# tbennun/capital

Hardware: NVIDIA H100
Metric: cholesky_tflops_fp64 (higher is better)
Workload: dtype f64

## Files before the change

capital_b200/csrc/common.cuh:

```cuda
#pragma once
#include <cuda.h>
#include <cuda_runtime.h>
#include <stdint.h>
#include <stdio.h>
#include <string.h>
#include <string>
#include <vector>
#include <map>
#include "../../include/capital_b200.h"

#define CAP_CUDA(call)                                                                                    \
  do {                                                                                                     \
    cudaError_t e__ = (call);                                                                              \
    if (e__ != cudaSuccess) {                                                                              \
      ctx->set_error(std::string(#call) + ": " + cudaGetErrorString(e__) + " (" + __FILE__ + ":" +         \
                     std::to_string(__LINE__) + ")");                                                      \
      return CAPITAL_ERR_CUDA;                                                                             \
    }                                                                                                      \
  } while (0)

#define CAP_TRY(call)                                  \
  do {                                                 \
    capital_status_t s__ = (call);                     \
    if (s__ != CAPITAL_OK) return s__;                 \
// ... 47 lines not shown
  int64_t tf32_min_k = 256;
  int64_t tf32_launches = 0;
  double tf32_flops = 0.0;
  std::vector<cudaEvent_t> prof_pool;
  size_t prof_used = 0;
  std::vector<ProfRec> prof_recs;
  capital_status_t prof_event(cudaEvent_t* out) {
    if (prof_used == prof_pool.size()) {
      cudaEvent_t e;
      if (cudaEventCreate(&e) != cudaSuccess) { err = "cudaEventCreate failed"; return CAPITAL_ERR_CUDA; }
      prof_pool.push_back(e);
    }
    *out = prof_pool[prof_used++];
    return CAPITAL_OK;
  }

  struct TlRec { cudaEvent_t e0, e1; int sid, kind; double a, b, c; };
  bool timeline = false;
  std::vector<TlRec> tl;
  std::vector<cudaEvent_t> tl_pool;
  size_t tl_used = 0;
  int stream_id(cudaStream_t st) const;
  int tl_begin(cudaStream_t st, int kind, double a = 0, double b = 0, double c = 0);
  void tl_end(cudaStream_t st, int idx);

  void set_error(const std::string& s) { err = s; }
  capital_status_t workspace(const std::string& name, size_t bytes, void** out);
};

capital_status_t gemm_tn_init(capital_ctx* ctx);
capital_status_t leaf_init(capital_ctx* ctx);
capital_status_t gemm_probe_dmma(capital_ctx* ctx, double* tflops, double* ms);

constexpr int GEMM_NCLS_MAX = 2;
constexpr int GEMM_XPEERS_MAX = 3;
struct GemmXDev {
  int mode, c, z;
  double* Cpeer[GEMM_XPEERS_MAX];
};
struct GemmOperands {
  int ncls = 1;
  const double* A[GEMM_NCLS_MAX] = {nullptr, nullptr};
  const double* B[GEMM_NCLS_MAX] = {nullptr, nullptr};
  int64_t lda = 0, ldb = 0;
};
capital_status_t gemm_tn_x(capital_ctx* ctx, cudaStream_t st, int64_t m, int64_t n, int64_t k, double alpha, const GemmOperands& ops,
                           double beta, double* C, int64_t ldc, int flags, int noff, const GemmXDev* x);
capital_status_t gemm_tn(capital_ctx* ctx, cudaStream_t st, int64_t m, int64_t n, int64_t k, double alpha, const double* A,
                         int64_t lda, const double* B, int64_t ldb, double beta, double* C, int64_t ldc, int flags);

capital_status_t gemm_tn_off(capital_ctx* ctx, cudaStream_t st, int64_t m, int64_t n, int64_t k, double alpha, const double* A,
                             int64_t lda, const double* B, int64_t ldb, double beta, double* C, int64_t ldc, int flags, int noff);
capital_status_t gemm_tn_splitk(capital_ctx* ctx, cudaStream_t st, int64_t m, int64_t n, int64_t k, double alpha, const double* A,
                                int64_t lda, const double* B, int64_t ldb, double* C, int64_t ldc, int flags);
capital_status_t gemm_tn_t(capital_ctx* ctx, cudaStream_t st, int64_t m, int64_t n, int64_t k, double alpha, const double* A, int64_t lda,
                           const double* B, int64_t ldb, double* C, int64_t ldc, double* Ct, int64_t ldct, int flags);

capital_status_t gemm_tf32_init(capital_ctx* ctx);
capital_status_t gemm_tn_tf32(capital_ctx* ctx, cudaStream_t st, int64_t m, int64_t n, int64_t k, double alpha, const double* A, int64_t lda,
                              const double* B, int64_t ldb, double beta, double* C, int64_t ldc, int flags, int passes);
capital_status_t gemm_tn_tf32_x(capital_ctx* ctx, cudaStream_t st, int64_t m, int64_t n, int64_t k, double alpha, const GemmOperands& ops,
                                double beta, double* C, int64_t ldc, int flags, int noff, int passes);
static inline bool trailing_uses_tf32(const capital_ctx* ctx, int64_t k) { return ctx->trailing_mode != 0 && k >= ctx->tf32_min_k; }

capital_status_t transpose_block(capital_ctx* ctx, cudaStream_t st, int64_t rows, int64_t cols, const double* src,
                                 int64_t lds, double* dst, int64_t ldd, double scale);
capital_status_t copy_block(capital_ctx* ctx, cudaStream_t st, int64_t rows, int64_t cols, const double* src, int64_t lds,
                            double* dst, int64_t ldd);
capital_status_t zero_block(capital_ctx* ctx, cudaStream_t st, int64_t rows, int64_t cols, double* dst, int64_t ldd);
capital_status_t zero_band(capital_ctx* ctx, cudaStream_t st, int64_t n, double* a, int64_t ld);
capital_status_t pack_upper(capital_ctx* ctx, cudaStream_t st, int64_t n, const double* src, int64_t lds, double* packed,
                            int zero_diag, int64_t col_begin = 0, int64_t col_end = -1);
capital_status_t unpack_upper(capital_ctx* ctx, cudaStream_t st, int64_t n, const double* packed, double* dst, int64_t ldd);
capital_status_t triu_copy(capital_ctx* ctx, cudaStream_t st, int64_t n, const double* src, int64_t lds, double* dst,
                           int64_t ldd, int zero_diag);
capital_status_t gen_symmetric(capital_ctx* ctx, cudaStream_t st, double* A, int64_t ld, int64_t lrows, int64_t lcols,
                               int64_t n_global, int x, int y, int d, int diag_dom);
capital_status_t gen_random(capital_ctx* ctx, cudaStream_t st, double* A, int64_t ld, int64_t lrows, int64_t lcols,
                            int64_t pad_rows, int64_t pad_cols, int64_t key);
capital_status_t sumsq_block(capital_ctx* ctx, cudaStream_t st, int64_t rows, int64_t cols, const double* a, int64_t ld,
                             int upper_mode, int x, int y, int d, double* out);
capital_status_t sub_identity_local(capital_ctx* ctx, cudaStream_t st, int64_t n, double* a, int64_t ld);

constexpr int LEAF_MAX = 64;
constexpr int BASECASE_MAX = 512;
capital_status_t basecase_cholinv(capital_ctx* ctx, cudaStream_t st, int nb, double* W, int64_t ldw, double* R, int64_t ldr,
                                  double* Ri, int64_t ldri, double* RiT, int64_t ldrit);
capital_status_t leaf_cholinv(capital_ctx* ctx, cudaStream_t st, int nb, const double* W, int64_t ldw, double* R, int64_t ldr,
                              double* Ri, int64_t ldri, double* RiT, int64_t ldrit);

struct CholinvHooks {
  void* user;
  capital_status_t (*need_cols)(void* user, cudaStream_t st, int64_t col_end);
  capital_status_t (*left_done)(void* user, cudaStream_t st, int64_t col_end, int depth);
  int64_t (*cols_waited)(void* user);
  capital_status_t (*right_done)(void* user, cudaStream_t st);
  capital_status_t (*inv_cols)(void* user, cudaStream_t st, int64_t col_end);
};
capital_status_t cholinv_local(capital_ctx* ctx, cudaStream_t st, int64_t n, double* W, int64_t ldw, double* R, int64_t ldr,
                               double* Ri, int64_t ldri, double* RiT, int64_t ldrit, bool complete_top, int64_t bc, int split,
                               const CholinvHooks* hooks = nullptr, bool allow_side = true);

static inline int64_t round_up(int64_t a, int64_t b) { return (a + b - 1) / b * b; }
static inline bool cholinv_node_splits(int64_t n, int64_t bc, int split) { return n > bc && (n >> split) >= split && (n >> split) > 0; }
static inline int64_t ceil_div(int64_t a, int64_t b) { return (a + b - 1) / b; }
```

capital_b200/csrc/gemm_tn.cu:

```cuda
#include "common.cuh"
#include <algorithm>

namespace {

struct GemmParams {
  int M, N, K;
  int rowoffA, rowoffB;
  int flags;
  int noff;
  int ksplit;
  int ncls;
  int gm, gn;
  double alpha, beta;
  double* C;
  long long ldc;
  double* Ct;
  long long ldct;
  double* kpart;
  long long kstride, ldk;
  int no_c;
  GemmXDev x;
};

struct GemmMaps {
  CUtensorMap a[GEMM_NCLS_MAX];
  CUtensorMap b[GEMM_NCLS_MAX];
};

__device__ __forceinline__ uint32_t smem_u32(const void* p) { return (uint32_t)__cvta_generic_to_shared(p); }

__device__ __forceinline__ void mbar_init(uint32_t bar, uint32_t count) {
  asm volatile("mbarrier.init.shared::cta.b64 [%0], %1;" ::"r"(bar), "r"(count) : "memory");
}
__device__ __forceinline__ void mbar_wait(uint32_t bar, uint32_t parity) {
  uint32_t ok;
  do {
    asm volatile(
        "{\n\t.reg .pred p;\n\t"
        "mbarrier.try_wait.parity.shared::cta.b64 p, [%1], %2;\n\t"
        "selp.u32 %0, 1, 0, p;\n\t}"
        : "=r"(ok)
        : "r"(bar), "r"(parity)
        : "memory");
  } while (!ok);
}
__device__ __forceinline__ void mbar_arrive(uint32_t bar) {
  asm volatile("mbarrier.arrive.shared::cta.b64 _, [%0];" ::"r"(bar) : "memory");
}
__device__ __forceinline__ void mbar_expect_tx(uint32_t bar, uint32_t bytes) {
  asm volatile("mbarrier.arrive.expect_tx.shared::cta.b64 _, [%0], %1;" ::"r"(bar), "r"(bytes) : "memory");
}
__device__ __forceinline__ void tma_load_2d(uint32_t dst, const CUtensorMap* map, uint32_t bar, int c0, int c1) {
  asm volatile(
      "cp.async.bulk.tensor.2d.shared::cluster.global.mbarrier::complete_tx::bytes [%0], [%1, {%3, %4}], [%2];" ::"r"(dst),
      "l"(map), "r"(bar), "r"(c0), "r"(c1)
      : "memory");
}
__device__ __forceinline__ void dmma16816(double& c0, double& c1, double& c2, double& c3, const double2 (&a0)[2], const double2 (&a1)[2],
                                          const double2 (&b)[2]) {
  asm("mma.sync.aligned.m16n8k16.row.col.f64.f64.f64.f64 {%0,%1,%2,%3}, {%4,%5,%6,%7,%8,%9,%10,%11}, {%12,%13,%14,%15}, {%0,%1,%2,%3};"
      : "+d"(c0), "+d"(c1), "+d"(c2), "+d"(c3)
      : "d"(a0[0].x), "d"(a1[0].x), "d"(a0[0].y), "d"(a1[0].y), "d"(a0[1].x), "d"(a1[1].x), "d"(a0[1].y), "d"(a1[1].y),
        "d"(b[0].x), "d"(b[0].y), "d"(b[1].x), "d"(b[1].y));
}

constexpr int BK = 16;

template <int BM, int BN, int WM, int WN, int STAGES, int MINB, int RC, int RP, int XMODE>
__global__ void __launch_bounds__(((BM / WM) * (BN / WN) + 4) * 32, MINB)
    gemm_tn_kernel(const __grid_constant__ GemmMaps maps, const GemmParams p) {
  constexpr int NWM = BM / WM, NWN = BN / WN, NCW = NWM * NWN;
  constexpr int FM = WM / 8, FN = WN / 8;
  static_assert(FM % 2 == 0, "DMMA.16x8x16 fragments pair the 8-row blocks of a warp tile");
  constexpr int A_BYTES = BM * 128, B_BYTES = BN * 128, STAGE_BYTES = A_BYTES + B_BYTES;

  extern __shared__ uint8_t smem_raw[];
  const int flags = p.flags;
  const int gm = p.gm, gn = p.gn;
  const int lin = (int)(blockIdx.x + gridDim.x * blockIdx.y);
  int tm, tn;
  if (flags & CAPITAL_GEMM_A_UPPER) { tm = gm - 1 - lin / gn; tn = lin % gn; }
  else if (flags & CAPITAL_GEMM_B_UPPER) { tn = gn - 1 - lin / gm; tm = lin % gm; }
  else if (flags & CAPITAL_GEMM_A_LOWER) { tm = lin / gn; tn = lin % gn; }
  else if (flags & CAPITAL_GEMM_B_LOWER) { tn = lin / gm; tm = lin % gm; }
  else { tm = lin % gm; tn = lin / gm; }
  if (XMODE == 2 && (tn % p.x.c) != p.x.z) return;
  const int m0 = tm * BM, n0 = tn * BN;
  const int n0g = n0 + p.noff;
  if ((flags & CAPITAL_GEMM_C_UPPER) && m0 > n0g + BN - 1) return;

  int kb = 0, ke = p.K;
  if (flags & CAPITAL_GEMM_A_UPPER) ke = min(ke, m0 + BM);
  if (flags & CAPITAL_GEMM_A_LOWER) kb = max(kb, m0);
  if (flags & CAPITAL_GEMM_B_UPPER) ke = min(ke, n0g + BN);
  if (flags & CAPITAL_GEMM_B_LOWER) kb = max(kb, n0g);
  kb &= ~(BK - 1);
  int nk = ke > kb ? (ke - kb + BK - 1) / BK : 0;
  if (nk == 0 && p.beta == 1.0 && p.ksplit <= 1) return;
  if (p.ksplit > 1) {
    const int per = (nk + p.ksplit - 1) / p.ksplit;
    const int t0 = min(nk, (int)blockIdx.z * per), t1 = min(nk, t0 + per);
    kb += t0 * BK;
    nk = t1 - t0;
    if (nk == 0) return;
  }
  const int niter = nk * p.ncls;

  const uint32_t raw_u32 = smem_u32(smem_raw);
  uint8_t* smem = smem_raw + (((raw_u32 + 1023u) & ~1023u) - raw_u32);
  const uint32_t smem_base = smem_u32(smem);
  const uint32_t full0 = smem_base + STAGES * STAGE_BYTES;
  const uint32_t empty0 = full0 + STAGES * 8;

  const int warp = threadIdx.x >> 5, lane = threadIdx.x & 31;
  if (threadIdx.x == 0) {
    for (int s = 0; s < STAGES; s++) {
      mbar_init(full0 + s * 8, 1);
      mbar_init(empty0 + s * 8, NCW);
    }
    asm volatile("fence.mbarrier_init.release.cluster;" ::: "memory");
    asm volatile("fence.proxy.async.shared::cta;" ::: "memory");
  }
  __syncthreads();

  if (warp >= NCW) {
    if (RC > 0) asm volatile("setmaxnreg.dec.sync.aligned.u32 %0;" ::"n"(RP));
    if (warp == NCW && lane == 0) {
      int it = 0;
      for (int cls = 0; cls < p.ncls; cls++) {
        const CUtensorMap* ma = cls ? &maps.a[1] : &maps.a[0];
        const CUtensorMap* mb = cls ? &maps.b[1] : &maps.b[0];
        for (int j = 0; j < nk; j++, it++) {
          const int s = it % STAGES;
          const uint32_t ph = (it / STAGES) & 1;
          mbar_wait(empty0 + s * 8, ph ^ 1);
          mbar_expect_tx(full0 + s * 8, STAGE_BYTES);
          const int kk = kb + j * BK;
          tma_load_2d(smem_base + s * STAGE_BYTES, ma, full0 + s * 8, p.rowoffA + kk, m0);
          tma_load_2d(smem_base + s * STAGE_BYTES + A_BYTES, mb, full0 + s * 8, p.rowoffB + kk, n0);
        }
      }
    }
    return;
  }

  if (RC > 0) asm volatile("setmaxnreg.inc.sync.aligned.u32 %0;" ::"n"(RC));
  const int wm = warp % NWM, wn = warp / NWM;
  const int g = lane >> 2, q = lane & 3;
// ... 336 lines not shown
```

capital_b200/csrc/leaf.cu:

```cuda
#include "common.cuh"
#include <cooperative_groups.h>
#include <stdlib.h>
#include <type_traits>
namespace cg = cooperative_groups;

namespace {
constexpr int LD = LEAF_MAX + 1;
constexpr int TLD = 68;
constexpr int TILE_DOUBLES = 64 * TLD;
constexpr int BC_CLUSTER = 8;

__device__ __forceinline__ double fast_rsqrt(double d) {
  if (!(d > 1e-30 && d < 1e30)) return rsqrt(d);
  double y = (double)rsqrtf((float)d);
  const double h = 0.5 * d;
  y = y * fma(-h, y * y, 1.5);
  y = y * fma(-h, y * y, 1.5);
  return y;
}

__device__ void leaf_factor_invert(int nb, double* __restrict__ a, double* __restrict__ r, double* __restrict__ t, int* info,
                                   int pivot_base) {
  const int tid = threadIdx.x, tx = tid & 15, ty = tid >> 4;
  for (int k = 0; k < nb; k++) {
    if (tid < 64 && tid >= k && tid < nb) {
      double d = a[k + k * LD];
      if (!(d > 0.0)) {
        if (tid == k) atomicCAS(info, 0, pivot_base + k + 1);
        d = 1.0;
      }
      const double rs = rsqrt(d);
      r[k + tid * LD] = (tid == k) ? d * rs : a[k + tid * LD] * rs;
    }
    __syncthreads();
#pragma unroll
    for (int ia = 0; ia < 4; ia++) {
      const int i = ty + 16 * ia;
      if (i > k && i < nb) {
        const double ri = r[k + i * LD];
#pragma unroll
        for (int jb = 0; jb < 4; jb++) {
          const int j = tx + 16 * jb;
          if (j >= i && j < nb) a[i + j * LD] -= ri * r[k + j * LD];
        }
      }
    }
    __syncthreads();
  }
#pragma unroll
  for (int ia = 0; ia < 4; ia++) {
    const int i = ty + 16 * ia;
#pragma unroll
    for (int jb = 0; jb < 4; jb++) {
      const int j = tx + 16 * jb;
      if (i < nb && j < nb) {
        if (i > j) r[i + j * LD] = 0.0;
        a[i + j * LD] = (i == j) ? 1.0 / r[i + i * LD] : 0.0;
      }
    }
  }
  __syncthreads();
  int lg = 0;
  for (int bs = 1; bs < nb; bs <<= 1, lg++) {
    const int span = 2 * bs;
    const int npairs = (nb + span - 1) / span;
    const int per = bs * bs, total = npairs * per;
    for (int idx = tid; idx < total; idx += 256) {
      const int p = idx >> (2 * lg), e = idx & (per - 1);
      const int li = e & (bs - 1), lj = e >> lg;
      const int o = p * span, i = o + li, j = o + bs + lj;
      if (j < nb) {
        double s = 0.0;
        const int kend = o + bs;
        for (int k = i; k < kend; k++) s += a[i + k * LD] * r[k + j * LD];
        t[i + j * LD] = s;
      }
    }
    __syncthreads();
    for (int idx = tid; idx < total; idx += 256) {
      const int p = idx >> (2 * lg), e = idx & (per - 1);
      const int li = e & (bs - 1), lj = e >> lg;
      const int o = p * span, i = o + li, j = o + bs + lj;
      if (j < nb) {
        double s = 0.0;
        for (int k = o + bs; k <= j; k++) s += t[i + k * LD] * a[k + j * LD];
        a[i + j * LD] = -s;
      }
    }
    __syncthreads();
  }
}

__device__ __forceinline__ void leaf_load(int nb, const double* W, long long ldw, double* __restrict__ a) {
  for (int idx = threadIdx.x; idx < nb * nb; idx += 256) {
    const int i = idx % nb, j = idx / nb;
    a[i + j * LD] = (i <= j) ? __ldcg(W + i + (long long)j * ldw) : 0.0;
  }
}
__device__ __forceinline__ void leaf_store(int nb, const double* a, const double* r, double* __restrict__ R,
                                           long long ldr, double* __restrict__ Ri, long long ldri, double* __restrict__ RiT,
                                           long long ldrit) {
  for (int idx = threadIdx.x; idx < nb * nb; idx += 256) {
    const int i = idx % nb, j = idx / nb;
    R[i + (long long)j * ldr] = r[i + j * LD];
    Ri[i + (long long)j * ldri] = a[i + j * LD];
  }
  if (RiT != nullptr) {
    for (int idx = threadIdx.x; idx < nb * nb; idx += 256) {
      const int j = idx % nb, i = idx / nb;
      RiT[j + (long long)i * ldrit] = a[i + j * LD];
    }
  }
}

__global__ void __launch_bounds__(256, 1)
    leaf_kernel(int nb, const double* W, long long ldw, double* __restrict__ R, long long ldr, double* __restrict__ Ri,
                long long ldri, double* __restrict__ RiT, long long ldrit, int* __restrict__ info) {
  extern __shared__ double sm[];
  double* a = sm;
  double* r = sm + LEAF_MAX * LD;
  double* t = sm + 2 * LEAF_MAX * LD;
  leaf_load(nb, W, ldw, a);
  __syncthreads();
  leaf_factor_invert(nb, a, r, t, info, 0);
  leaf_store(nb, a, r, R, ldr, Ri, ldri, RiT, ldrit);
}

__device__ __forceinline__ void dmma884(double& c0, double& c1, double a, double b) {
  asm("mma.sync.aligned.m8n8k4.row.col.f64.f64.f64.f64 {%0,%1}, {%2}, {%3}, {%0,%1};" : "+d"(c0), "+d"(c1) : "d"(a), "d"(b));
}
__device__ __forceinline__ void tile_load(double* __restrict__ dst, const double* src, long long ld) {
  const int k2 = (threadIdx.x & 31) * 2, c0 = threadIdx.x >> 5;
  double2 v[8];
#pragma unroll
  for (int r = 0; r < 8; r++) v[r] = __ldcg(reinterpret_cast<const double2*>(src + k2 + (long long)(c0 + 8 * r) * ld));
#pragma unroll
  for (int r = 0; r < 8; r++) *reinterpret_cast<double2*>(dst + (c0 + 8 * r) * TLD + k2) = v[r];
}
__device__ __forceinline__ void tile_mma(double (&acc)[4][2][2], const double* As, const double* Bs) {
  const int lane = threadIdx.x & 31, w = threadIdx.x >> 5, g = lane >> 2, q = lane & 3;
  const double* ap = As + ((w & 1) * 32 + g) * TLD + q;
  const double* bp = Bs + ((w >> 1) * 16 + g) * TLD + q;
#pragma unroll 4
  for (int k0 = 0; k0 < 64; k0 += 4) {
    double af[4], bf[2];
#pragma unroll
    for (int i = 0; i < 4; i++) af[i] = ap[i * 8 * TLD + k0];
#pragma unroll
    for (int j = 0; j < 2; j++) bf[j] = bp[j * 8 * TLD + k0];
#pragma unroll
    for (int i = 0; i < 4; i++)
#pragma unroll
      for (int j = 0; j < 2; j++) dmma884(acc[i][j][0], acc[i][j][1], af[i], bf[j]);
  }
}
__device__ __forceinline__ void acc_zero(double (&acc)[4][2][2]) {
#pragma unroll
  for (int i = 0; i < 4; i++)
#pragma unroll
    for (int j = 0; j < 2; j++) acc[i][j][0] = acc[i][j][1] = 0.0;
}
#define TILE_ROW(i) ((w & 1) * 32 + (i) * 8 + g)
#define TILE_COL(j, e) ((w >> 1) * 16 + (j) * 8 + 2 * q + (e))
__device__ __forceinline__ void acc_to_smem_colmajor(const double (&acc)[4][2][2], double* __restrict__ sC, double scale) {
  const int lane = threadIdx.x & 31, w = threadIdx.x >> 5, g = lane >> 2, q = lane & 3;
#pragma unroll
  for (int i = 0; i < 4; i++)
#pragma unroll
    for (int j = 0; j < 2; j++)
#pragma unroll
      for (int e = 0; e < 2; e++) sC[TILE_COL(j, e) * TLD + TILE_ROW(i)] = scale * acc[i][j][e];
}
__device__ __forceinline__ void acc_to_smem_rowmajor(const double (&acc)[4][2][2], double* __restrict__ sC, double scale) {
  const int lane = threadIdx.x & 31, w = threadIdx.x >> 5, g = lane >> 2, q = lane & 3;
#pragma unroll
  for (int i = 0; i < 4; i++)
#pragma unroll
    for (int j = 0; j < 2; j++)
#pragma unroll
      for (int e = 0; e < 2; e++) sC[TILE_ROW(i) * TLD + TILE_COL(j, e)] = scale * acc[i][j][e];
}
template <bool ACCUM>
__device__ __forceinline__ void tile_store(double* __restrict__ dst, long long ld, const double* sC) {
  const int r2 = (threadIdx.x & 31) * 2, c0 = threadIdx.x >> 5;
#pragma unroll
  for (int r = 0; r < 8; r++) {
    const int c = c0 + 8 * r;
    double2 v = *reinterpret_cast<const double2*>(sC + c * TLD + r2);
    double2* p = reinterpret_cast<double2*>(dst + r2 + (long long)c * ld);
    if (ACCUM) { const double2 o = __ldcg(p); v.x += o.x; v.y += o.y; }
    *p = v;
  }
}
__device__ __forceinline__ void tile_store_from_rowmajor(double* __restrict__ dst, long long ld, const double* sCr) {
  const int c2 = (threadIdx.x & 31) * 2, r0 = threadIdx.x >> 5;
#pragma unroll
  for (int r = 0; r < 8; r++) {
    const int row = r0 + 8 * r;
    const double2 v = *reinterpret_cast<const double2*>(sCr + row * TLD + c2);
    *reinterpret_cast<double2*>(dst + c2 + (long long)row * ld) = v;
  }
}

__device__ __forceinline__ double shfl_d(double v, int src) { return __shfl_sync(0xffffffffu, v, src); }

template <int I, int END, int STEP = 1, typename F>
__device__ __forceinline__ void static_for(F&& f) {
  if constexpr (I < END) {
    f(std::integral_constant<int, I>{});
    static_for<I + STEP, END, STEP>(f);
  }
}

__device__ __forceinline__ void warp_potrf_trtri_32(double (&c)[32], double* __restrict__ sRb, double* __restrict__ sXb, double* __restrict__ sXTb,
                                                    double* __restrict__ ub, int lane, int* info, int pivot_base, long long* dbg2) {
  double myrs = 0.0;
  if (dbg2 && lane == 0) dbg2[0] = clock64();
  double a = shfl_d(c[0], 0), l = shfl_d(c[0], 1), b = shfl_d(c[1], 1);
  static_for<0, 32, 2>([&](auto kc) {
    constexpr int k = decltype(kc)::value;
    if (!(a > 0.0)) { if (lane == k) atomicCAS(info, 0, pivot_base + k + 1); a = 1.0; }
    double det = fma(b, a, -(l * l));
    if (!(det > 0.0)) { if (lane == k + 1) atomicCAS(info, 0, pivot_base + k + 2); det = 1.0; }
    const double ra = fast_rsqrt(a), rdet = fast_rsqrt(det);
    const double sa = a * ra, lk = l * ra, rs2 = sa * rdet;
    const double u0 = (lane > k) ? c[k] * ra : (lane == k ? sa : 0.0);
    const double t1 = fma(-lk, u0, c[k + 1]);
    const double u1 = (lane > k + 1) ? t1 * rs2 : (lane == k + 1 ? det * rdet * ra : 0.0);
    c[k] = u0;
    c[k + 1] = u1;
    if (lane == k) myrs = ra;
    if (lane == k + 1) myrs = rs2;
    double* row0 = ub + (k & 2) * 32;
    double* row1 = row0 + 32;
    row0[lane] = u0;
    row1[lane] = u1;
    __syncwarp();
    if constexpr (k + 2 < 32) {
      c[k + 2] = fma(-row1[k + 2], u1, fma(-row0[k + 2], u0, c[k + 2]));
      c[k + 3] = fma(-row1[k + 3], u1, fma(-row0[k + 3], u0, c[k + 3]));
      a = shfl_d(c[k + 2], k + 2);
      l = shfl_d(c[k + 2], k + 3);
      b = shfl_d(c[k + 3], k + 3);
      static_for<k + 4, 32>([&](auto ic) {
        constexpr int i = decltype(ic)::value;
        c[i] = fma(-row1[i], u1, fma(-row0[i], u0, c[i]));
      });
    }
  });
  if (dbg2 && lane == 0) dbg2[1] = clock64();
#pragma unroll
  for (int i = 0; i < 32; i++) sRb[lane * TLD + i] = c[i];
  __syncwarp();
  const int g16 = lane >> 4, jl = lane & 15, base = 16 * g16;
  double xl[16];
  static_for<0, 16>([&](auto rc_) { constexpr int r = decltype(rc_)::value; xl[r] = (r == jl) ? myrs : 0.0; });
  static_for<0, 15>([&](auto sc) {
    constexpr int il = 14 - decltype(sc)::value;
    const double rsi = shfl_d(myrs, base + il);
    double s0 = 0.0, s1 = 0.0, s2 = 0.0, s3 = 0.0;
    static_for<il + 1, 16>([&](auto tc) {
      constexpr int t = decltype(tc)::value;
      const double rit = sRb[(base + t) * TLD + base + il];
      if constexpr ((t & 3) == 0) s0 = fma(rit, xl[t], s0);
      else if constexpr ((t & 3) == 1) s1 = fma(rit, xl[t], s1);
      else if constexpr ((t & 3) == 2) s2 = fma(rit, xl[t], s2);
      else s3 = fma(rit, xl[t], s3);
    });
    if (jl > il) xl[il] = -rsi * ((s0 + s1) + (s2 + s3));
  });
  double* xs = ub + 128;
  double* ts = ub + 128 + 512;
  static_for<0, 16>([&](auto rc_) {
    constexpr int r = decltype(rc_)::value;
    xs[lane * 16 + r] = xl[r];
    sXb[lane * TLD + base + r] = xl[r];
    sXTb[(base + r) * TLD + lane] = xl[r];
  });
  __syncwarp();
  {
    double rc[16], tr[8];
    static_for<0, 16>([&](auto tc) { constexpr int t = decltype(tc)::value; rc[t] = sRb[(16 + jl) * TLD + t]; });
    static_for<0, 8>([&](auto rr) {
      constexpr int r = decltype(rr)::value;
      const int i = 8 * g16 + r;
      double s = 0.0;
      static_for<0, 16>([&](auto tc) {
        constexpr int t = decltype(tc)::value;
        s = fma(xs[t * 16 + i], rc[t], s);
      });
      tr[r] = s;
      ts[jl * 16 + i] = s;
    });
    __syncwarp();
    double xc[16];
    static_for<0, 16>([&](auto tc) { constexpr int t = decltype(tc)::value; xc[t] = xs[(16 + jl) * 16 + t]; });
    static_for<0, 8>([&](auto rr) {
      constexpr int r = decltype(rr)::value;
      const int i = 8 * g16 + r;
      double s = 0.0;
      static_for<0, 16>([&](auto tc) {
        constexpr int t = decltype(tc)::value;
        s = fma(ts[t * 16 + i], xc[t], s);
      });
      sXb[(16 + jl) * TLD + i] = -s;
      sXTb[i * TLD + 16 + jl] = -s;
    });
    (void)tr;
  }
  __syncwarp();
  if (dbg2 && lane == 0) dbg2[2] = clock64();
}

__device__ __forceinline__ void mma32(double (&acc)[2][2], const double* As, int ar, const double* Bs, int bc, int k0) {
  const int lane = threadIdx.x & 31, w = threadIdx.x >> 5, g = lane >> 2, q = lane & 3;
  const double* ap = As + (ar + (w & 3) * 8 + g) * TLD + k0 + q;
  const double* bp = Bs + (bc + (w >> 2) * 16 + g) * TLD + k0 + q;
#pragma unroll
  for (int k = 0; k < 32; k += 4) {
    const double a = ap[k], b0 = bp[k], b1 = bp[8 * TLD + k];
    dmma884(acc[0][0], acc[0][1], a, b0);
    dmma884(acc[1][0], acc[1][1], a, b1);
  }
}
#define M32_ROW ((w & 3) * 8 + g)
#define M32_COL(j, e) ((w >> 2) * 16 + (j) * 8 + 2 * q + (e))

__device__ void leaf64_fast(double* __restrict__ sA, double* __restrict__ sR, double* __restrict__ sX, double* __restrict__ sXT,
                            double* __restrict__ ub, int* info, int pivot_base, long long* dbg2 = nullptr) {
  const int tid = threadIdx.x, lane = tid & 31, w = tid >> 5, g = lane >> 2, q = lane & 3;
  for (int idx = tid; idx < 64 * 64; idx += 256) {
    const int r = idx & 63, cidx = idx >> 6;
    sR[cidx * TLD + r] = 0.0; sX[cidx * TLD + r] = 0.0; sXT[cidx * TLD + r] = 0.0;
  }
  __syncthreads();
  double c[32];
#pragma unroll 1
  for (int half = 0; half < 2; half++) {
    const int o = half * 32;
    if (half == 1) {
      double acc[2][2] = {{0.0, 0.0}, {0.0, 0.0}};
      mma32(acc, sX, 0, sA, 32, 0);
#pragma unroll
      for (int j = 0; j < 2; j++)
#pragma unroll
        for (int e = 0; e < 2; e++) sR[(32 + M32_COL(j, e)) * TLD + M32_ROW] = acc[j][e];
      __syncthreads();
      double acc2[2][2] = {{0.0, 0.0}, {0.0, 0.0}};
      mma32(acc2, sR + 32 * TLD, 0, sR + 32 * TLD, 0, 0);
#pragma unroll
      for (int j = 0; j < 2; j++)
#pragma unroll
        for (int e = 0; e < 2; e++) sA[(32 + M32_COL(j, e)) * TLD + 32 + M32_ROW] -= acc2[j][e];
      __syncthreads();
    }
    if (w == 0) {
#pragma unroll
      for (int i = 0; i < 32; i++) c[i] = sA[(o + lane) * TLD + o + i];
      warp_potrf_trtri_32(c, sR + o * TLD + o, sX + o * TLD + o, sXT + o * TLD + o, ub, lane, info, pivot_base + o,
                          (dbg2 && half == 0) ? dbg2 : nullptr);
      if (dbg2 && half == 0 && lane == 0) dbg2[3] = clock64();
    }
    __syncthreads();
  }
  {
    double acc[2][2] = {{0.0, 0.0}, {0.0, 0.0}};
    mma32(acc, sXT, 0, sR, 32, 0);
    __syncthreads();
#pragma unroll
    for (int j = 0; j < 2; j++)
#pragma unroll
      for (int e = 0; e < 2; e++) sA[M32_ROW * TLD + 32 + M32_COL(j, e)] = acc[j][e];
    __syncthreads();
    double acc2[2][2] = {{0.0, 0.0}, {0.0, 0.0}};
    mma32(acc2, sA, 0, sX, 32, 32);
#pragma unroll
    for (int j = 0; j < 2; j++)
#pragma unroll
      for (int e = 0; e < 2; e++) {
        const double v = -acc2[j][e];
        sX[(32 + M32_COL(j, e)) * TLD + M32_ROW] = v;
        sXT[M32_ROW * TLD + 32 + M32_COL(j, e)] = v;
      }
  }
  __syncthreads();
}

__global__ void __cluster_dims__(BC_CLUSTER, 1, 1) __launch_bounds__(256, 1)
    basecase_kernel(int nb, double* __restrict__ W, long long ldw, double* __restrict__ R, long long ldr, double* __restrict__ Ri,
                    long long ldri, double* __restrict__ RiT, long long ldrit, int* __restrict__ info, long long* __restrict__ dbg) {
  extern __shared__ __align__(16) double sm[];
  double* sA = sm;
  double* sB = sm + TILE_DOUBLES;
  double* sT = sm + 2 * TILE_DOUBLES;
  cg::cluster_group cluster = cg::this_cluster();
  const int rank = (int)cluster.block_rank();
  const int T = nb >> 6;
  double acc[4][2][2];
  int dbgi = 0;
#define DBG_STAMP() do { if (dbg && rank == 0 && threadIdx.x == 0) dbg[dbgi++] = clock64(); } while (0)
  DBG_STAMP();

  double* sU = sm + 3 * TILE_DOUBLES;
  auto do_leaf = [&](int jb) {
    const long long o = (long long)jb * 64;
    __syncthreads();
    tile_load(sA, W + o + o * ldw, ldw);
    __syncthreads();
    if (dbg && jb == 0 && threadIdx.x == 0) dbg[20] = clock64();
    leaf64_fast(sA, sB, sT, sU, sm + 4 * TILE_DOUBLES, info, jb * 64, (dbg && jb == 0) ? dbg + 24 : nullptr);
    if (dbg && jb == 0 && threadIdx.x == 0) dbg[21] = clock64();
    tile_store<false>(R + o + o * ldr, ldr, sB);
    tile_store<false>(Ri + o + o * ldri, ldri, sT);
    tile_store<false>(RiT + o + o * ldrit, ldrit, sU);
    __syncthreads();
  };
  auto do_trailing = [&](int jb, int i, int j) {
    const long long o = (long long)jb * 64;
    __syncthreads();
    tile_load(sA, R + o + (long long)i * 64 * ldr, ldr);
    tile_load(sB, R + o + (long long)j * 64 * ldr, ldr);
    __syncthreads();
    acc_zero(acc);
    tile_mma(acc, sA, sB);
    acc_to_smem_colmajor(acc, sT, -1.0);
    __syncthreads();
    tile_store<true>(W + (long long)i * 64 + (long long)j * 64 * ldw, ldw, sT);
  };

  if (rank == 0) do_leaf(0);
  DBG_STAMP();
  __threadfence();
  cluster.sync();
  DBG_STAMP();
  for (int jb = 0; jb < T; jb++) {
    const long long o = (long long)jb * 64;
    int work = 0;
    for (int j = jb + 1; j < T; j++, work++) {
      if (work % BC_CLUSTER != rank) continue;
      __syncthreads();
      tile_load(sA, Ri + o + o * ldri, ldri);
      tile_load(sB, W + o + (long long)j * 64 * ldw, ldw);
      __syncthreads();
      acc_zero(acc);
      tile_mma(acc, sA, sB);
      acc_to_smem_colmajor(acc, sT, 1.0);
      __syncthreads();
      tile_store<false>(R + o + (long long)j * 64 * ldr, ldr, sT);
    }
    if (jb == 0) DBG_STAMP();
    __threadfence();
    cluster.sync();
    if (jb == 0) DBG_STAMP();
    if (jb + 1 < T) {
      const int leaf_rank = (jb + 1) % BC_CLUSTER;
      if (rank == leaf_rank) {
        do_trailing(jb, jb + 1, jb + 1);
        __threadfence_block();
        do_leaf(jb + 1);
      } else {
        const int slot = rank > leaf_rank ? rank - 1 : rank;
        work = 0;
        for (int j = jb + 1; j < T; j++)
          for (int i = jb + 1; i <= j; i++) {
            if (i == jb + 1 && j == jb + 1) continue;
            if (work++ % (BC_CLUSTER - 1) != slot) continue;
            do_trailing(jb, i, j);
          }
      }
    }
    if (jb == 0) DBG_STAMP();
    __threadfence();
    cluster.sync();
    if (jb == 0) DBG_STAMP();
  }
  DBG_STAMP();
  {
    int work = 0;
    for (int j = 0; j < T; j++)
      for (int i = j + 1; i < T; i++, work++) {
        if (work % BC_CLUSTER != rank) continue;
        for (int idx = threadIdx.x; idx < 4096; idx += 256)
          R[(long long)i * 64 + (idx & 63) + ((long long)j * 64 + (idx >> 6)) * ldr] = 0.0;
      }
  }
  for (int bs = 1; bs < T; bs <<= 1) {
    const int span = 2 * bs;
    int work = 0;
    for (int o = 0; o + bs < T; o += span) {
      const int jend = min(o + span, T);
      for (int j = o + bs; j < jend; j++)
        for (int i = o; i < o + bs; i++, work++) {
          if (work % BC_CLUSTER != rank) continue;
          acc_zero(acc);
          for (int k = i; k < o + bs; k++) {
            __syncthreads();
            tile_load(sA, RiT + (long long)k * 64 + (long long)i * 64 * ldrit, ldrit);
            tile_load(sB, R + (long long)k * 64 + (long long)j * 64 * ldr, ldr);
            __syncthreads();
            tile_mma(acc, sA, sB);
          }
          __syncthreads();
          acc_to_smem_rowmajor(acc, sT, 1.0);
          __syncthreads();
          tile_store_from_rowmajor(W + (long long)j * 64 + (long long)i * 64 * ldw, ldw, sT);
        }
    }
    __threadfence();
    cluster.sync();
    work = 0;
    for (int o = 0; o + bs < T; o += span) {
      const int jend = min(o + span, T);
      for (int j = o + bs; j < jend; j++)
        for (int i = o; i < o + bs; i++, work++) {
          if (work % BC_CLUSTER != rank) continue;
          acc_zero(acc);
          for (int k = o + bs; k <= j; k++) {
            __syncthreads();
            tile_load(sA, W + (long long)k * 64 + (long long)i * 64 * ldw, ldw);
            tile_load(sB, Ri + (long long)k * 64 + (long long)j * 64 * ldri, ldri);
            __syncthreads();
            tile_mma(acc, sA, sB);
          }
          __syncthreads();
          acc_to_smem_colmajor(acc, sA, -1.0);
          acc_to_smem_rowmajor(acc, sB, -1.0);
          __syncthreads();
          tile_store<false>(Ri + (long long)i * 64 + (long long)j * 64 * ldri, ldri, sA);
          tile_store_from_rowmajor(RiT + (long long)j * 64 + (long long)i * 64 * ldrit, ldrit, sB);
        }
    }
    __threadfence();
    cluster.sync();
  }
  DBG_STAMP();
}
}

namespace {
constexpr int LEAF_SMEM = 3 * LEAF_MAX * LD * (int)sizeof(double);
constexpr int BASECASE_SMEM = (4 * TILE_DOUBLES + 128 + 512 + 256) * (int)sizeof(double);
}
capital_status_t leaf_init(capital_ctx* ctx) {
  CAP_CUDA(cudaFuncSetAttribute(leaf_kernel, cudaFuncAttributeMaxDynamicSharedMemorySize, LEAF_SMEM));
  CAP_CUDA(cudaFuncSetAttribute(basecase_kernel, cudaFuncAttributeMaxDynamicSharedMemorySize, BASECASE_SMEM));
  return CAPITAL_OK;
}

capital_status_t leaf_cholinv(capital_ctx* ctx, cudaStream_t st, int nb, const double* W, int64_t ldw, double* R, int64_t ldr, double* Ri,
                              int64_t ldri, double* RiT, int64_t ldrit) {
  if (nb <= 0) return CAPITAL_OK;
  if (nb > LEAF_MAX) return CAPITAL_ERR_INVALID;
  constexpr int smem = LEAF_SMEM;
  const int tli = ctx->tl_begin(st, 4, nb);
  leaf_kernel<<<1, 256, smem, st>>>(nb, W, ldw, R, ldr, Ri, ldri, RiT, ldrit, ctx->d_info);
  ctx->tl_end(st, tli);
  ctx->counters.kernel_launches++;
  ctx->counters.leaf_launches++;
  CAP_CUDA(cudaGetLastError());
  return CAPITAL_OK;
}

capital_status_t basecase_cholinv(capital_ctx* ctx, cudaStream_t st, int nb, double* W, int64_t ldw, double* R, int64_t ldr, double* Ri,
                                  int64_t ldri, double* RiT, int64_t ldrit) {
  if (nb % 64 != 0 || nb < 64 || nb > BASECASE_MAX || RiT == nullptr) return CAPITAL_ERR_INVALID;
  constexpr int smem = BASECASE_SMEM;
  long long* dbg = nullptr;
  if (getenv("CAPITAL_BC_DEBUG")) {
    CAP_TRY(ctx->workspace("bc_dbg", 64 * sizeof(long long), (void**)&dbg));
    CAP_CUDA(cudaMemsetAsync(dbg, 0, 64 * sizeof(long long), st));
  }
  const int tli = ctx->tl_begin(st, 3, nb);
  basecase_kernel<<<BC_CLUSTER, 256, smem, st>>>(nb, W, ldw, R, ldr, Ri, ldri, RiT, ldrit, ctx->d_info, dbg);
  ctx->tl_end(st, tli);
  if (dbg) {
    long long h[32];
    CAP_CUDA(cudaMemcpyAsync(h, dbg, sizeof(h), cudaMemcpyDeviceToHost, st));
    CAP_CUDA(cudaStreamSynchronize(st));
    fprintf(stderr, "[bc nb=%d] leaf0=%lld bar=%lld panel0=%lld bar=%lld trail0+leaf1=%lld bar=%lld | chol_total=%lld inverse=%lld total=%lld cycles\n", nb,
            h[1] - h[0], h[2] - h[1], h[3] - h[2], h[4] - h[3], h[5] - h[4], h[6] - h[5], h[7] - h[0], h[8] - h[7], h[8] - h[0]);
    fprintf(stderr, "   leaf64: load=%lld total=%lld | warp32: pre=%lld potrf=%lld trtri=%lld store=%lld\n", h[20] - h[0], h[21] - h[20], h[24] - h[20],
            h[25] - h[24], h[26] - h[25], h[27] - h[26]);
  }
  ctx->counters.kernel_launches++;
  ctx->counters.leaf_launches++;
  CAP_CUDA(cudaGetLastError());
  return CAPITAL_OK;
}
```

Measured before the change: 30.73.

## Use m16n8k16 DMMA in basecase, overlap leaf with split barrier and early inverse stages

The basecase kernel's tile GEMMs move from m8n8k4 to m16n8k16 FP64 MMA with vectorized double2 shared loads, and the tile leading dimension changes from 68 to 66. The next diagonal leaf's trailing update and factorization now run on the lead CTA between split cluster arrive/wait barriers, so it overlaps the panel work on the other CTAs. Inverse-merge stages for the first half of the blocks are interleaved into the Cholesky loop on the non-lead CTAs, and the remaining stages are rescheduled. This adds scheduling complexity and a risk of race or correctness issues in exchange for fewer serialized barriers and better tensor-core throughput.

Measured after the change: 31.47 (median of 6 runs). 2.4% higher.

```diff
diff --git a/capital_b200/csrc/common.cuh b/capital_b200/csrc/common.cuh
--- a/capital_b200/csrc/common.cuh
+++ b/capital_b200/csrc/common.cuh
@@ -153,6 +153,14 @@
                              int upper_mode, int x, int y, int d, double* out);
 capital_status_t sub_identity_local(capital_ctx* ctx, cudaStream_t st, int64_t n, double* a, int64_t ld);
 
+__device__ __forceinline__ void dmma16816(double& c0, double& c1, double& c2, double& c3, const double2 (&a0)[2], const double2 (&a1)[2],
+                                          const double2 (&b)[2]) {
+  asm("mma.sync.aligned.m16n8k16.row.col.f64.f64.f64.f64 {%0,%1,%2,%3}, {%4,%5,%6,%7,%8,%9,%10,%11}, {%12,%13,%14,%15}, {%0,%1,%2,%3};"
+      : "+d"(c0), "+d"(c1), "+d"(c2), "+d"(c3)
+      : "d"(a0[0].x), "d"(a1[0].x), "d"(a0[0].y), "d"(a1[0].y), "d"(a0[1].x), "d"(a1[1].x), "d"(a0[1].y), "d"(a1[1].y),
+        "d"(b[0].x), "d"(b[0].y), "d"(b[1].x), "d"(b[1].y));
+}
+
 constexpr int LEAF_MAX = 64;
 constexpr int BASECASE_MAX = 512;
 capital_status_t basecase_cholinv(capital_ctx* ctx, cudaStream_t st, int nb, double* W, int64_t ldw, double* R, int64_t ldr,
diff --git a/capital_b200/csrc/gemm_tn.cu b/capital_b200/csrc/gemm_tn.cu
--- a/capital_b200/csrc/gemm_tn.cu
+++ b/capital_b200/csrc/gemm_tn.cu
@@ -56,14 +56,6 @@
       "l"(map), "r"(bar), "r"(c0), "r"(c1)
       : "memory");
 }
-__device__ __forceinline__ void dmma16816(double& c0, double& c1, double& c2, double& c3, const double2 (&a0)[2], const double2 (&a1)[2],
-                                          const double2 (&b)[2]) {
-  asm("mma.sync.aligned.m16n8k16.row.col.f64.f64.f64.f64 {%0,%1,%2,%3}, {%4,%5,%6,%7,%8,%9,%10,%11}, {%12,%13,%14,%15}, {%0,%1,%2,%3};"
-      : "+d"(c0), "+d"(c1), "+d"(c2), "+d"(c3)
-      : "d"(a0[0].x), "d"(a1[0].x), "d"(a0[0].y), "d"(a1[0].y), "d"(a0[1].x), "d"(a1[1].x), "d"(a0[1].y), "d"(a1[1].y),
-        "d"(b[0].x), "d"(b[0].y), "d"(b[1].x), "d"(b[1].y));
-}
-
 constexpr int BK = 16;
 
 template <int BM, int BN, int WM, int WN, int STAGES, int MINB, int RC, int RP, int XMODE>
diff --git a/capital_b200/csrc/leaf.cu b/capital_b200/csrc/leaf.cu
--- a/capital_b200/csrc/leaf.cu
+++ b/capital_b200/csrc/leaf.cu
@@ -6,7 +6,7 @@
 
 namespace {
 constexpr int LD = LEAF_MAX + 1;
-constexpr int TLD = 68;
+constexpr int TLD = 66;
 constexpr int TILE_DOUBLES = 64 * TLD;
 constexpr int BC_CLUSTER = 8;
 
@@ -126,9 +126,7 @@
   leaf_store(nb, a, r, R, ldr, Ri, ldri, RiT, ldrit);
 }
 
-__device__ __forceinline__ void dmma884(double& c0, double& c1, double a, double b) {
-  asm("mma.sync.aligned.m8n8k4.row.col.f64.f64.f64.f64 {%0,%1}, {%2}, {%3}, {%0,%1};" : "+d"(c0), "+d"(c1) : "d"(a), "d"(b));
-}
+__device__ __forceinline__ double2 lds2(const double* p) { return *reinterpret_cast<const double2*>(p); }
 __device__ __forceinline__ void tile_load(double* __restrict__ dst, const double* src, long long ld) {
   const int k2 = (threadIdx.x & 31) * 2, c0 = threadIdx.x >> 5;
   double2 v[8];
@@ -137,48 +135,60 @@
 #pragma unroll
   for (int r = 0; r < 8; r++) *reinterpret_cast<double2*>(dst + (c0 + 8 * r) * TLD + k2) = v[r];
 }
-__device__ __forceinline__ void tile_mma(double (&acc)[4][2][2], const double* As, const double* Bs) {
+__device__ __forceinline__ void tile_mma(double (&acc)[2][2][4], const double* As, const double* Bs) {
   const int lane = threadIdx.x & 31, w = threadIdx.x >> 5, g = lane >> 2, q = lane & 3;
-  const double* ap = As + ((w & 1) * 32 + g) * TLD + q;
-  const double* bp = Bs + ((w >> 1) * 16 + g) * TLD + q;
-#pragma unroll 4
-  for (int k0 = 0; k0 < 64; k0 += 4) {
-    double af[4], bf[2];
-#pragma unroll
-    for (int i = 0; i < 4; i++) af[i] = ap[i * 8 * TLD + k0];
-#pragma unroll
-    for (int j = 0; j < 2; j++) bf[j] = bp[j * 8 * TLD + k0];
-#pragma unroll
-    for (int i = 0; i < 4; i++)
-#pragma unroll
-      for (int j = 0; j < 2; j++) dmma884(acc[i][j][0], acc[i][j][1], af[i], bf[j]);
-  }
-}
-__device__ __forceinline__ void acc_zero(double (&acc)[4][2][2]) {
-#pragma unroll
-  for (int i = 0; i < 4; i++)
-#pragma unroll
-    for (int j = 0; j < 2; j++) acc[i][j][0] = acc[i][j][1] = 0.0;
-}
-#define TILE_ROW(i) ((w & 1) * 32 + (i) * 8 + g)
+  const double* ap = As + ((w & 1) * 32 + g) * TLD + 4 * q;
+  const double* bp = Bs + ((w >> 1) * 16 + g) * TLD + 4 * q;
+#pragma unroll 2
+  for (int k0 = 0; k0 < 64; k0 += 16) {
+    double2 a[2][2][2], b[2][2];
+#pragma unroll
+    for (int i = 0; i < 2; i++)
+#pragma unroll
+      for (int r = 0; r < 2; r++)
+#pragma unroll
+        for (int h = 0; h < 2; h++) a[i][r][h] = lds2(ap + (i * 16 + r * 8) * TLD + k0 + 2 * h);
+#pragma unroll
+    for (int j = 0; j < 2; j++)
+#pragma unroll
+      for (int h = 0; h < 2; h++) b[j][h] = lds2(bp + j * 8 * TLD + k0 + 2 * h);
+#pragma unroll
+    for (int i = 0; i < 2; i++)
+#pragma unroll
+      for (int j = 0; j < 2; j++) dmma16816(acc[i][j][0], acc[i][j][1], acc[i][j][2], acc[i][j][3], a[i][0], a[i][1], b[j]);
+  }
+}
+__device__ __forceinline__ void acc_zero(double (&acc)[2][2][4]) {
+#pragma unroll
+  for (int i = 0; i < 2; i++)
+#pragma unroll
+    for (int j = 0; j < 2; j++)
+#pragma unroll
+      for (int e = 0; e < 4; e++) acc[i][j][e] = 0.0;
+}
+#define TILE_ROW(i, h) ((w & 1) * 32 + (i) * 16 + (h) * 8 + g)
 #define TILE_COL(j, e) ((w >> 1) * 16 + (j) * 8 + 2 * q + (e))
-__device__ __forceinline__ void acc_to_smem_colmajor(const double (&acc)[4][2][2], double* __restrict__ sC, double scale) {
+__device__ __forceinline__ void acc_to_smem_colmajor(const double (&acc)[2][2][4], double* __restrict__ sC, double scale) {
   const int lane = threadIdx.x & 31, w = threadIdx.x >> 5, g = lane >> 2, q = lane & 3;
 #pragma unroll
-  for (int i = 0; i < 4; i++)
+  for (int i = 0; i < 2; i++)
 #pragma unroll
     for (int j = 0; j < 2; j++)
 #pragma unroll
-      for (int e = 0; e < 2; e++) sC[TILE_COL(j, e) * TLD + TILE_ROW(i)] = scale * acc[i][j][e];
-}
-__device__ __forceinline__ void acc_to_smem_rowmajor(const double (&acc)[4][2][2], double* __restrict__ sC, double scale) {
+      for (int h = 0; h < 2; h++)
+#pragma unroll
+        for (int e = 0; e < 2; e++) sC[TILE_COL(j, e) * TLD + TILE_ROW(i, h)] = scale * acc[i][j][2 * h + e];
+}
+__device__ __forceinline__ void acc_to_smem_rowmajor(const double (&acc)[2][2][4], double* __restrict__ sC, double scale) {
   const int lane = threadIdx.x & 31, w = threadIdx.x >> 5, g = lane >> 2, q = lane & 3;
 #pragma unroll
-  for (int i = 0; i < 4; i++)
+  for (int i = 0; i < 2; i++)
 #pragma unroll
     for (int j = 0; j < 2; j++)
 #pragma unroll
-      for (int e = 0; e < 2; e++) sC[TILE_ROW(i) * TLD + TILE_COL(j, e)] = scale * acc[i][j][e];
+      for (int h = 0; h < 2; h++)
+#pragma unroll
+        for (int e = 0; e < 2; e++) sC[TILE_ROW(i, h) * TLD + TILE_COL(j, e)] = scale * acc[i][j][2 * h + e];
 }
 template <bool ACCUM>
 __device__ __forceinline__ void tile_store(double* __restrict__ dst, long long ld, const double* sC) {
@@ -312,19 +322,19 @@
   if (dbg2 && lane == 0) dbg2[2] = clock64();
 }
 
-__device__ __forceinline__ void mma32(double (&acc)[2][2], const double* As, int ar, const double* Bs, int bc, int k0) {
+__device__ __forceinline__ void mma32(double (&acc)[4], const double* As, int ar, const double* Bs, int bc, int k0) {
   const int lane = threadIdx.x & 31, w = threadIdx.x >> 5, g = lane >> 2, q = lane & 3;
-  const double* ap = As + (ar + (w & 3) * 8 + g) * TLD + k0 + q;
-  const double* bp = Bs + (bc + (w >> 2) * 16 + g) * TLD + k0 + q;
-#pragma unroll
-  for (int k = 0; k < 32; k += 4) {
-    const double a = ap[k], b0 = bp[k], b1 = bp[8 * TLD + k];
-    dmma884(acc[0][0], acc[0][1], a, b0);
-    dmma884(acc[1][0], acc[1][1], a, b1);
-  }
-}
-#define M32_ROW ((w & 3) * 8 + g)
-#define M32_COL(j, e) ((w >> 2) * 16 + (j) * 8 + 2 * q + (e))
+  const double* ap = As + (ar + (w & 1) * 16 + g) * TLD + k0 + 4 * q;
+  const double* bp = Bs + (bc + (w >> 1) * 8 + g) * TLD + k0 + 4 * q;
+#pragma unroll
+  for (int k = 0; k < 32; k += 16) {
+    const double2 a0[2] = {lds2(ap + k), lds2(ap + k + 2)}, a1[2] = {lds2(ap + 8 * TLD + k), lds2(ap + 8 * TLD + k + 2)};
+    const double2 b[2] = {lds2(bp + k), lds2(bp + k + 2)};
+    dmma16816(acc[0], acc[1], acc[2], acc[3], a0, a1, b);
+  }
+}
+#define M32_ROW(h) ((w & 1) * 16 + (h) * 8 + g)
+#define M32_COL(e) ((w >> 1) * 8 + 2 * q + (e))
 
 __device__ void leaf64_fast(double* __restrict__ sA, double* __restrict__ sR, double* __restrict__ sX, double* __restrict__ sXT,
                             double* __restrict__ ub, int* info, int pivot_base, long long* dbg2 = nullptr) {
@@ -339,19 +349,19 @@
   for (int half = 0; half < 2; half++) {
     const int o = half * 32;
     if (half == 1) {
-      double acc[2][2] = {{0.0, 0.0}, {0.0, 0.0}};
+      double acc[4] = {0.0, 0.0, 0.0, 0.0};
       mma32(acc, sX, 0, sA, 32, 0);
 #pragma unroll
-      for (int j = 0; j < 2; j++)
-#pragma unroll
-        for (int e = 0; e < 2; e++) sR[(32 + M32_COL(j, e)) * TLD + M32_ROW] = acc[j][e];
-      __syncthreads();
-      double acc2[2][2] = {{0.0, 0.0}, {0.0, 0.0}};
+      for (int h = 0; h < 2; h++)
+#pragma unroll
+        for (int e = 0; e < 2; e++) sR[(32 + M32_COL(e)) * TLD + M32_ROW(h)] = acc[2 * h + e];
+      __syncthreads();
+      double acc2[4] = {0.0, 0.0, 0.0, 0.0};
       mma32(acc2, sR + 32 * TLD, 0, sR + 32 * TLD, 0, 0);
 #pragma unroll
-      for (int j = 0; j < 2; j++)
-#pragma unroll
-        for (int e = 0; e < 2; e++) sA[(32 + M32_COL(j, e)) * TLD + 32 + M32_ROW] -= acc2[j][e];
+      for (int h = 0; h < 2; h++)
+#pragma unroll
+        for (int e = 0; e < 2; e++) sA[(32 + M32_COL(e)) * TLD + 32 + M32_ROW(h)] -= acc2[2 * h + e];
       __syncthreads();
     }
     if (w == 0) {
@@ -364,27 +374,30 @@
     __syncthreads();
   }
   {
-    double acc[2][2] = {{0.0, 0.0}, {0.0, 0.0}};
+    double acc[4] = {0.0, 0.0, 0.0, 0.0};
     mma32(acc, sXT, 0, sR, 32, 0);
     __syncthreads();
 #pragma unroll
-    for (int j = 0; j < 2; j++)
-#pragma unroll
-      for (int e = 0; e < 2; e++) sA[M32_ROW * TLD + 32 + M32_COL(j, e)] = acc[j][e];
-    __syncthreads();
-    double acc2[2][2] = {{0.0, 0.0}, {0.0, 0.0}};
+    for (int h = 0; h < 2; h++)
+#pragma unroll
+      for (int e = 0; e < 2; e++) sA[M32_ROW(h) * TLD + 32 + M32_COL(e)] = acc[2 * h + e];
+    __syncthreads();
+    double acc2[4] = {0.0, 0.0, 0.0, 0.0};
     mma32(acc2, sA, 0, sX, 32, 32);
 #pragma unroll
-    for (int j = 0; j < 2; j++)
+    for (int h = 0; h < 2; h++)
 #pragma unroll
       for (int e = 0; e < 2; e++) {
-        const double v = -acc2[j][e];
-        sX[(32 + M32_COL(j, e)) * TLD + M32_ROW] = v;
-        sXT[M32_ROW * TLD + 32 + M32_COL(j, e)] = v;
+        const double v = -acc2[2 * h + e];
+        sX[(32 + M32_COL(e)) * TLD + M32_ROW(h)] = v;
+        sXT[M32_ROW(h) * TLD + 32 + M32_COL(e)] = v;
       }
   }
   __syncthreads();
 }
+
+__device__ __forceinline__ void cluster_arrive() { asm volatile("barrier.cluster.arrive.release.aligned;" ::: "memory"); }
+__device__ __forceinline__ void cluster_wait() { asm volatile("barrier.cluster.wait.acquire.aligned;" ::: "memory"); }
 
 __global__ void __cluster_dims__(BC_CLUSTER, 1, 1) __launch_bounds__(256, 1)
     basecase_kernel(int nb, double* __restrict__ W, long long ldw, double* __restrict__ R, long long ldr, double* __restrict__ Ri,
@@ -393,20 +406,17 @@
   double* sA = sm;
   double* sB = sm + TILE_DOUBLES;
   double* sT = sm + 2 * TILE_DOUBLES;
+  double* sU = sm + 3 * TILE_DOUBLES;
   cg::cluster_group cluster = cg::this_cluster();
   const int rank = (int)cluster.block_rank();
   const int T = nb >> 6;
-  double acc[4][2][2];
+  double acc[2][2][4];
   int dbgi = 0;
 #define DBG_STAMP() do { if (dbg && rank == 0 && threadIdx.x == 0) dbg[dbgi++] = clock64(); } while (0)
   DBG_STAMP();
 
-  double* sU = sm + 3 * TILE_DOUBLES;
   auto do_leaf = [&](int jb) {
     const long long o = (long long)jb * 64;
-    __syncthreads();
-    tile_load(sA, W + o + o * ldw, ldw);
-    __syncthreads();
     if (dbg && jb == 0 && threadIdx.x == 0) dbg[20] = clock64();
     leaf64_fast(sA, sB, sT, sU, sm + 4 * TILE_DOUBLES, info, jb * 64, (dbg && jb == 0) ? dbg + 24 : nullptr);
     if (dbg && jb == 0 && threadIdx.x == 0) dbg[21] = clock64();
@@ -427,17 +437,86 @@
     __syncthreads();
     tile_store<true>(W + (long long)i * 64 + (long long)j * 64 * ldw, ldw, sT);
   };
-
-  if (rank == 0) do_leaf(0);
+  auto store_inverse_tile = [&](int i, int j) {
+    __syncthreads();
+    acc_to_smem_colmajor(acc, sA, -1.0);
+    acc_to_smem_rowmajor(acc, sU, -1.0);
+    __syncthreads();
+    tile_store<false>(Ri + (long long)i * 64 + (long long)j * 64 * ldri, ldri, sA);
+    tile_store_from_rowmajor(RiT + (long long)j * 64 + (long long)i * 64 * ldrit, ldrit, sU);
+  };
+  auto inv_job = [&](int phase, int o, int bs, int i, int j) {
+    acc_zero(acc);
+    if (phase != 2) {
+      for (int k = i; k < o + bs; k++) {
+        __syncthreads();
+        tile_load(sA, RiT + (long long)k * 64 + (long long)i * 64 * ldrit, ldrit);
+        tile_load(sB, R + (long long)k * 64 + (long long)j * 64 * ldr, ldr);
+        __syncthreads();
+        tile_mma(acc, sA, sB);
+      }
+      __syncthreads();
+      acc_to_smem_rowmajor(acc, sT, 1.0);
+      __syncthreads();
+      if (phase == 1) {
+        tile_store_from_rowmajor(W + (long long)j * 64 + (long long)i * 64 * ldw, ldw, sT);
+        return;
+      }
+      tile_load(sB, Ri + (long long)j * 64 + (long long)j * 64 * ldri, ldri);
+      __syncthreads();
+      acc_zero(acc);
+      tile_mma(acc, sT, sB);
+    } else {
+      for (int k = o + bs; k <= j; k++) {
+        __syncthreads();
+        tile_load(sA, W + (long long)k * 64 + (long long)i * 64 * ldw, ldw);
+        tile_load(sB, Ri + (long long)k * 64 + (long long)j * 64 * ldri, ldri);
+        __syncthreads();
+        tile_mma(acc, sA, sB);
+      }
+    }
+    store_inverse_tile(i, j);
+  };
+  auto inv_stage = [&](int phase, int bs, int ob, int oe, int slot, int nslots) {
+    int work = 0;
+    for (int o = ob; o < oe && o + bs < T; o += 2 * bs) {
+      const int jend = min(o + 2 * bs, T);
+      for (int j = o + bs; j < jend; j++)
+        for (int i = o; i < o + bs; i++, work++)
+          if (work % nslots == slot) inv_job(phase, o, bs, i, j);
+    }
+  };
+  int H = 1;
+  while (2 * H < T) H *= 2;
+  auto early_stage = [&](int s, int slot, int nslots) {
+    for (int bs = 1; bs < H; bs *= 2) {
+      if (bs == 1) { if (s-- == 0) return inv_stage(0, 1, 0, H, slot, nslots); }
+      else {
+        if (s-- == 0) return inv_stage(1, bs, 0, H, slot, nslots);
+        if (s-- == 0) return inv_stage(2, bs, 0, H, slot, nslots);
+      }
+    }
+    if (s == 0) inv_stage(1, H, 0, 1, slot, nslots);
+  };
+  int n_early = 1;
+  for (int bs = 1; bs < H; bs *= 2) n_early += bs == 1 ? 1 : 2;
+  int early_done = 0;
+
+  if (rank == 0) {
+    tile_load(sA, W, ldw);
+    __syncthreads();
+    do_leaf(0);
+  }
   DBG_STAMP();
   __threadfence();
   cluster.sync();
   DBG_STAMP();
   for (int jb = 0; jb < T; jb++) {
     const long long o = (long long)jb * 64;
-    int work = 0;
-    for (int j = jb + 1; j < T; j++, work++) {
-      if (work % BC_CLUSTER != rank) continue;
+    const int leaf_rank = (jb + 1) % BC_CLUSTER;
+    const bool lead = jb + 1 < T && rank == leaf_rank;
+    const int slot = rank > leaf_rank ? rank - 1 : rank;
+    auto panel_tile = [&](int j) {
       __syncthreads();
       tile_load(sA, Ri + o + o * ldri, ldri);
       tile_load(sB, W + o + (long long)j * 64 * ldw, ldw);
@@ -447,27 +526,51 @@
       acc_to_smem_colmajor(acc, sT, 1.0);
       __syncthreads();
       tile_store<false>(R + o + (long long)j * 64 * ldr, ldr, sT);
+    };
+    if (lead) {
+      panel_tile(jb + 1);
+    } else {
+      int work = 0;
+      for (int j = jb + 2; j < T; j++, work++)
+        if (work % (BC_CLUSTER - 1) == slot) panel_tile(j);
     }
     if (jb == 0) DBG_STAMP();
     __threadfence();
-    cluster.sync();
+    cluster_arrive();
+    if (lead) {
+      const long long o1 = o + 64;
+      tile_load(sA, W + o1 + o1 * ldw, ldw);
+      acc_zero(acc);
+      tile_mma(acc, sT, sT);
+      __syncthreads();
+      {
+        const int lane = threadIdx.x & 31, w = threadIdx.x >> 5, g = lane >> 2, q = lane & 3;
+#pragma unroll
+        for (int i = 0; i < 2; i++)
+#pragma unroll
+          for (int j = 0; j < 2; j++)
+#pragma unroll
+            for (int h = 0; h < 2; h++)
+#pragma unroll
+              for (int e = 0; e < 2; e++) sA[TILE_COL(j, e) * TLD + TILE_ROW(i, h)] -= acc[i][j][2 * h + e];
+      }
+      __syncthreads();
+      do_leaf(jb + 1);
+    }
+    cluster_wait();
     if (jb == 0) DBG_STAMP();
     if (jb + 1 < T) {
-      const int leaf_rank = (jb + 1) % BC_CLUSTER;
-      if (rank == leaf_rank) {
-        do_trailing(jb, jb + 1, jb + 1);
-        __threadfence_block();
-        do_leaf(jb + 1);
-      } else {
-        const int slot = rank > leaf_rank ? rank - 1 : rank;
-        work = 0;
+      if (!lead) {
+        int work = 0;
         for (int j = jb + 1; j < T; j++)
           for (int i = jb + 1; i <= j; i++) {
             if (i == jb + 1 && j == jb + 1) continue;
             if (work++ % (BC_CLUSTER - 1) != slot) continue;
             do_trailing(jb, i, j);
           }
-      }
+        if (jb >= H - 1 && early_done < n_early) early_stage(early_done, slot, BC_CLUSTER - 1);
+      }
+      if (jb >= H - 1 && early_done < n_early) early_done++;
     }
     if (jb == 0) DBG_STAMP();
     __threadfence();
@@ -484,55 +587,27 @@
           R[(long long)i * 64 + (idx & 63) + ((long long)j * 64 + (idx >> 6)) * ldr] = 0.0;
       }
   }
-  for (int bs = 1; bs < T; bs <<= 1) {
-    const int span = 2 * bs;
-    int work = 0;
-    for (int o = 0; o + bs < T; o += span) {
-      const int jend = min(o + span, T);
-      for (int j = o + bs; j < jend; j++)
-        for (int i = o; i < o + bs; i++, work++) {
-          if (work % BC_CLUSTER != rank) continue;
-          acc_zero(acc);
-          for (int k = i; k < o + bs; k++) {
-            __syncthreads();
-            tile_load(sA, RiT + (long long)k * 64 + (long long)i * 64 * ldrit, ldrit);
-            tile_load(sB, R + (long long)k * 64 + (long long)j * 64 * ldr, ldr);
-            __syncthreads();
-            tile_mma(acc, sA, sB);
-          }
-          __syncthreads();
-          acc_to_smem_rowmajor(acc, sT, 1.0);
-          __syncthreads();
-          tile_store_from_rowmajor(W + (long long)j * 64 + (long long)i * 64 * ldw, ldw, sT);
-        }
-    }
+  auto stage_barrier = [&]() {
     __threadfence();
     cluster.sync();
-    work = 0;
-    for (int o = 0; o + bs < T; o += span) {
-      const int jend = min(o + span, T);
-      for (int j = o + bs; j < jend; j++)
-        for (int i = o; i < o + bs; i++, work++) {
-          if (work % BC_CLUSTER != rank) continue;
-          acc_zero(acc);
-          for (int k = o + bs; k <= j; k++) {
-            __syncthreads();
-            tile_load(sA, W + (long long)k * 64 + (long long)i * 64 * ldw, ldw);
-            tile_load(sB, Ri + (long long)k * 64 + (long long)j * 64 * ldri, ldri);
-            __syncthreads();
-            tile_mma(acc, sA, sB);
-          }
-          __syncthreads();
-          acc_to_smem_colmajor(acc, sA, -1.0);
-          acc_to_smem_rowmajor(acc, sB, -1.0);
-          __syncthreads();
-          tile_store<false>(Ri + (long long)i * 64 + (long long)j * 64 * ldri, ldri, sA);
-          tile_store_from_rowmajor(RiT + (long long)j * 64 + (long long)i * 64 * ldrit, ldrit, sB);
-        }
-    }
-    __threadfence();
-    cluster.sync();
-  }
+  };
+  for (; early_done < n_early; early_done++) {
+    early_stage(early_done, rank, BC_CLUSTER);
+    stage_barrier();
+  }
+  for (int bs = 1; bs < H; bs *= 2) {
+    if (H + bs >= T) break;
+    if (bs == 1) {
+      inv_stage(0, 1, H, T, rank, BC_CLUSTER);
+      stage_barrier();
+    } else {
+      inv_stage(1, bs, H, T, rank, BC_CLUSTER);
+      stage_barrier();
+      inv_stage(2, bs, H, T, rank, BC_CLUSTER);
+      stage_barrier();
+    }
+  }
+  inv_stage(2, H, 0, 1, rank, BC_CLUSTER);
   DBG_STAMP();
 }
 }
@@ -577,7 +652,7 @@
     long long h[32];
     CAP_CUDA(cudaMemcpyAsync(h, dbg, sizeof(h), cudaMemcpyDeviceToHost, st));
     CAP_CUDA(cudaStreamSynchronize(st));
-    fprintf(stderr, "[bc nb=%d] leaf0=%lld bar=%lld panel0=%lld bar=%lld trail0+leaf1=%lld bar=%lld | chol_total=%lld inverse=%lld total=%lld cycles\n", nb,
+    fprintf(stderr, "[bc nb=%d] leaf0=%lld bar=%lld panel0=%lld bar=%lld trail0+leaf1=%lld bar=%lld | chol_total=%lld inverse_tail=%lld total=%lld cycles\n", nb,
             h[1] - h[0], h[2] - h[1], h[3] - h[2], h[4] - h[3], h[5] - h[4], h[6] - h[5], h[7] - h[0], h[8] - h[7], h[8] - h[0]);
     fprintf(stderr, "   leaf64: load=%lld total=%lld | warp32: pre=%lld potrf=%lld trtri=%lld store=%lld\n", h[20] - h[0], h[21] - h[20], h[24] - h[20],
             h[25] - h[24], h[26] - h[25], h[27] - h[26]);
```
